# luofeisg/OpenKE-PuTransE

Hardware: AMD Instinct MI355X
Metric: training triples/sec (pos+neg) (higher is better)
Workload: dtype fp32; 1 GPU; C2 TransE fb15k237-shaped dim 200 p2 sgd lr 1 margin 5 batch 2000 neg 25 bern 1 filter 1 threads 8; global_batch=52000, parallelism=single

## Files before the change

include/putranse.h:

```cpp
#ifndef PUTRANSE_H
#define PUTRANSE_H
#include <stdint.h>

#ifdef __cplusplus
extern "C" {
#endif

enum {
    PT_OK = 0,
    PT_EINVAL = 1,
    PT_EIO = 2,
    PT_ENOMEM = 3,
    PT_EHIP = 4,
    PT_ESTATE = 5,
    PT_ENOTSUP = 6
};
const char *pt_last_error(void);
int pt_version(void);

typedef struct pt_graph pt_graph;
int pt_graph_load(const char *in_path, pt_graph **out);
int pt_set_count_header(int on);
int pt_get_count_header(void);
int pt_graph_free(pt_graph *g);
// ... 31 lines not shown

typedef struct pt_trainer pt_trainer;
int pt_trainer_create(const pt_model_desc *m, pt_trainer **out);
int pt_trainer_free(pt_trainer *t);
int pt_trainer_update_desc(pt_trainer *t, const pt_model_desc *m);
int pt_trainer_step(pt_trainer *t, pt_sampler *sampler, int64_t bs, int64_t neg, int64_t bern, int64_t filter,
                    const int64_t *d_batch_h, const int64_t *d_batch_t, const int64_t *d_batch_r, float *d_loss,
                    void *stream);
int pt_trainer_run(pt_trainer *t, pt_sampler *sampler, int64_t bs, int64_t neg, int64_t bern, int64_t filter,
                   int64_t steps, float *d_losses, void *stream);
int pt_trainer_fused_supported(const pt_trainer *t, int64_t bs, int64_t neg);

int pt_trainer_set_sampling(pt_trainer *t, int32_t path, int64_t parts);
int pt_trainer_set_positive_caps(pt_trainer *t, int32_t ent_cap, int32_t rel_cap);
int pt_trainer_positive_caps(const pt_trainer *t, int32_t *ent_cap, int32_t *rel_cap);
int pt_trainer_set_sample_split(pt_trainer *t, int64_t head);
int pt_trainer_set_deterministic(pt_trainer *t, int32_t on);
int pt_trainer_get_deterministic(const pt_trainer *t);

enum { PT_LOSS_MARGIN = 0, PT_LOSS_SIGMOID = 1 };
typedef struct {
    int32_t kind;
    int32_t adv;
    float temperature;
    int32_t score_margin_flag;
    float score_margin;
} pt_loss_desc;
int pt_trainer_set_loss(pt_trainer *t, const pt_loss_desc *loss);
typedef struct {
    float *ent_m, *rel_m, *norm_m;
// ... 13 lines not shown
                           const int64_t *d_batch_r, int64_t steps, float *d_loss, float *ms2, void *stream);

int pt_trainer_run_timed(pt_trainer *t, pt_sampler *sampler, int64_t bs, int64_t neg, int64_t bern, int64_t filter,
                         int64_t steps, float *d_losses, float *ms4, void *stream);
enum { PT_PATH_TWO_PASS = 0, PT_PATH_FUSED = 1, PT_PATH_PART = 2, PT_PATH_SAMPLED = 3 };
int pt_trainer_last_path(const pt_trainer *t);
int pt_trainer_set_step_apply(pt_trainer *t, int32_t on);
int pt_trainer_step_apply(const pt_trainer *t);
int pt_trainer_set_slot_scale(pt_trainer *t, int32_t on);
int pt_trainer_slot_scale(const pt_trainer *t);
int pt_trainer_sample_csr(pt_trainer *t, pt_sampler *sampler, int64_t bs, int64_t neg, int64_t bern, int64_t filter,
                          int64_t calls, int32_t path, int32_t *h_pos, int32_t *h_neg, int32_t *h_dst,
                          int32_t *h_start, void *stream);
int pt_trainer_positive_slots(pt_trainer *t, int64_t calls, int32_t *h_pdst, int32_t *h_pstart, int32_t *stored,
                              void *stream);

int pt_score(const pt_model_desc *m, int32_t mode, const int64_t *d_h, const int64_t *d_t, const int64_t *d_r,
             int64_t n, float *d_out, void *stream);

int pt_score_queries(const pt_model_desc *m, int32_t side, const int64_t *d_qh, const int64_t *d_qt,
                     const int64_t *d_qr, int64_t nq, float *d_out, void *stream);
int pt_score_rows(const pt_model_desc *m, int32_t side, const int64_t *d_qh, const int64_t *d_qt,
                  const int64_t *d_qr, int64_t nq, float *d_out, void *stream);
int pt_lp_metrics(const int64_t *rank_head, const int64_t *frank_head, const int64_t *rank_tail,
                  const int64_t *frank_tail, int64_t n, float *metrics);

typedef struct pt_universe pt_universe;
int pt_universe_build(const pt_graph *g, int64_t seed, int64_t threads, int64_t triple_constraint,
                      float balance, pt_universe **out);
int pt_universe_free(pt_universe *u);
// ... 163 lines not shown
```

openke-putranse_amd/csrc/apply.hip:

```cpp
#include <hip/hip_runtime.h>

#include <cstdint>

#include "device.h"
#include "graph.h"
#include "kernels.h"
#include "rng.h"

namespace pt {
namespace dev {
using pt::CsrWork;

struct ApplyTable {
    float *w, *acc, *grad;
    int *flag;
    int64_t rows;
    int jacobian;
    const int *start;
    const int *pstart;
};
struct ApplyParams {
    ApplyTable t[3];
    int ntab;
    int64_t dim;
    int opt;
    float lr;
    uint64_t *states;
    int64_t threads, bs, dpp;
    float *loss;
    const float *lpart;
    float margin, inv_count;
    int loss_assign;
    const float *contrib;
};

__device__ __forceinline__ void apply_block0(const ApplyParams &A) {
    const int lane = (int)threadIdx.x;
    if (A.states) advance_states(A.states, A.threads, A.bs, A.dpp, lane);
    if (A.loss && A.lpart) {
        float s = 0.f;
        for (int64_t i0 = lane; i0 < A.bs; i0 += 64 * 8) {
            float v[8];
#pragma unroll
            for (int u = 0; u < 8; ++u) v[u] = i0 + u * 64 < A.bs ? A.lpart[i0 + u * 64] : 0.f;
#pragma unroll
            for (int u = 0; u < 8; ++u) s += v[u];
        }
        s = gsum<64>(s);
// ... 61 lines not shown
        for (int i = 0; i < Vec::N; ++i) {
            a.x[i] = a.x[i] + g.x[i] * g.x[i];
            x.x[i] = x.x[i] + (-A.lr) * g.x[i] / (sqrtf(a.x[i]) + 1e-10f);
        }
        vstore(a, T.acc + row * D, D, lane);
    }
    vstore(x, T.w + row * D, D, lane);
    if (flagged) {
        Vec z;
        vzero(z);
        vstore(z, T.grad + row * D, D, lane);
        if (lane == 0) T.flag[row] = 0;
    }
}

template <int G, int VEC, int KCH, int NC>
__global__ __launch_bounds__(256) void k_apply_buf(ApplyParams A) {
    using Vec = V<G, VEC, KCH>;
    constexpr int GPB = 256 / G;
    const int lane = threadIdx.x % G;
    const int64_t gi = uni<G>((int32_t)(blockIdx.x * GPB + threadIdx.x / G));
    if (blockIdx.x == 0 && threadIdx.x < 64) apply_block0(A);
    const int D = (int)A.dim;
    const uint32_t rowb = (uint32_t)D * 4u;
    int64_t row = gi;
    int ti = 0;
    while (ti < A.ntab && row >= A.t[ti].rows) {
        row -= A.t[ti].rows;
        ++ti;
    }
    const bool live = ti < A.ntab;
    int flag = 0, c0 = 0, c1 = 0, p0 = 0, p1 = 0;
    Vec x, g, a;
#pragma unroll
    for (int once = 0; once < 1; ++once) {
        if (!live) continue;
        const ApplyTable &T = A.t[ti];
        const uint32_t tb = (uint32_t)T.rows * rowb;
        bload(x, make_rsrc(T.w, tb), (uint32_t)row * rowb, D, lane);
        if (A.opt != 0) bload(a, make_rsrc(T.acc, tb), (uint32_t)row * rowb, D, lane);
        flag = T.flag[row];
        if (T.start) {
            c0 = T.start[row];
            c1 = T.start[row + 1];
        }
        if (T.pstart) {
            p0 = T.pstart[row];
            p1 = T.pstart[row + 1];
        }
    }
    int len = 0, n0 = 0;
#pragma unroll
    for (int once = 0; once < 1; ++once) {
        if (!live) continue;
        const ApplyTable &T = A.t[ti];
        bload(g, make_rsrc(T.grad, (uint32_t)T.rows * rowb), flag ? (uint32_t)row * rowb : kOob, D, lane);
        n0 = c1 - c0;
        len = n0 + (p1 - p0);
    }
    const auto c_rs = make_rsrc(A.contrib, 0x7fffffffu);
    for (int j = 0; j < len; j += NC) {
        Vec c[NC];
#pragma unroll
        for (int q = 0; q < NC; ++q) {
            const int i = j + q;
            const int r = i < n0 ? c0 + i : p0 + (i - n0);
            bload(c[q], c_rs, i < len ? (uint32_t)r * rowb : kOob, D, lane);
        }
#pragma unroll
        for (int q = 0; q < NC; ++q)
#pragma unroll
            for (int i = 0; i < Vec::N; ++i) g.x[i] += c[q].x[i];
    }
#pragma unroll
    for (int once = 0; once < 1; ++once) {
        if (!live || (!flag && len == 0)) continue;
        const ApplyTable &T = A.t[ti];
        const uint32_t tb = (uint32_t)T.rows * rowb;
        Vec gg;
        if (T.jacobian) {
            const float n = sqrtf(vdot(x, x));
            vnormalize_bwd(x, n, g, gg);
        } else {
            gg = g;
        }
        if (A.opt == 0) {
#pragma unroll
// ... 21 lines not shown
hipError_t launch_apply(const StepParams &P, const StepWorkspace &W, uint64_t *states, int64_t threads, int64_t bs,
                        int64_t dpp, float *loss, hipStream_t st, const CsrWork *csr) {
    const Shape s = pick_shape(P.dim);
    dev::ApplyParams A{};
    A.ntab = 0;
    const int ent_j = P.model == 0 && P.norm_flag;
    const dev::ApplyTable ent{P.ent, P.ent_acc, W.gent, W.fent, P.ent_total, ent_j, csr ? csr->start : nullptr,
                              csr ? csr->pstart : nullptr};
    const dev::ApplyTable rel{P.rel, P.rel_acc, W.grel, W.frel, P.rel_total, P.norm_flag, nullptr,
                              csr && csr->pstart ? csr->pstart + P.ent_total : nullptr};
    A.t[A.ntab++] = csr ? rel : ent;
    A.t[A.ntab++] = csr ? ent : rel;
    if (P.model == 1)
        A.t[A.ntab++] = dev::ApplyTable{P.normv, P.norm_acc, W.gnorm, W.fnorm, P.rel_total, 1, nullptr, nullptr};
    A.contrib = csr ? csr->contrib : nullptr;
    A.dim = P.dim;
    A.opt = P.opt;
    A.lr = P.lr;
    A.states = states;
    A.threads = threads;
    A.bs = bs;
    A.dpp = dpp;
    A.loss = loss;
    A.lpart = W.lpart;
    A.margin = P.margin;
    A.inv_count = P.inv_count;
    A.loss_assign = P.loss_assign;
    int64_t rows = 0;
    for (int i = 0; i < A.ntab; ++i) rows += A.t[i].rows;
    const bool buf = P.dim % 4 == 0 && offsets_fit31(P, csr ? csr_con_rows(P.batch_size, P.neg) : 0);
    const int64_t gpb = 256 / s.G;
    const dim3 grid((unsigned)((rows + gpb - 1) / gpb)), block(256);
    hipError_t e = hipErrorInvalidValue;
    for_shape(s, [&](auto sh) {
        using T = decltype(sh);
        if constexpr (T::VEC == 4) {
            constexpr int NC = T::G == 64 && T::KCH == 1 ? 8 : 4;
            if (buf) {
                hipLaunchKernelGGL((dev::k_apply_buf<T::G, 4, T::KCH, NC>), grid, block, 0, st, A);
                e = hipGetLastError();
                return;
            }
        }
        hipLaunchKernelGGL((dev::k_apply<T::G, T::VEC, T::KCH>), grid, block, 0, st, A);
        e = hipGetLastError();
    });
    return e;
}

}
```

openke-putranse_amd/csrc/kernels.h:

```cpp
#pragma once
#include <hip/hip_runtime.h>

#include <cstdint>
#include <type_traits>

#include "graph.h"

namespace pt {

struct StepParams {
    int model, p_norm, norm_flag, opt;
    float lr, margin;
    int64_t ent_total, rel_total, dim;
    float *ent, *rel, *normv;
    float *ent_acc, *rel_acc, *norm_acc;
    int64_t batch_size, neg;
    float inv_count;
    int loss_assign = 0;
    float *ent_t = nullptr, *rel_t = nullptr;
    float *ent_t_acc = nullptr, *rel_t_acc = nullptr;
    float phase_div = 0.f;
};

struct StepWorkspace {
// ... 5 lines not shown
};

struct CsrWork {
    int4 *pos = nullptr;
    int32_t *neg = nullptr;
    int32_t *off = nullptr;
    int32_t *cnt = nullptr;
    int32_t *start = nullptr;
    float *contrib = nullptr;
    int32_t *tick = nullptr;
    int rank_only = 0;
    int64_t cnt_stride = 0, start_stride = 0;
    int4 *pdst = nullptr;
    int32_t *pstart = nullptr;
    int64_t pstart_stride = 0;
};

inline CsrWork csr_view(const CsrWork &w, int64_t call, int64_t bs, int64_t neg) {
    CsrWork v = w;
    v.pos = w.pos + call * bs;
    v.neg = w.neg + call * bs * neg;
    v.off = w.off + call * bs * neg;
    v.cnt = w.cnt + call * w.cnt_stride;
    v.start = w.start + call * w.start_stride;
    v.pdst = w.pdst + call * bs;
    v.pstart = w.pstart + call * w.pstart_stride;
    return v;
}

struct LpUniverseDev {
// ... 73 lines not shown
hipError_t launch_sample_part(const DeviceGraph &g, uint64_t *states, int64_t threads, int64_t bs, int64_t neg,
                              int bern, int filter, int64_t calls, int64_t parts, int64_t n, const CsrWork &w,
                              hipStream_t st);
bool sample_sort_prepare(int64_t bs, int64_t neg, int64_t n, int64_t start_stride);
bool sample_part_fits(int64_t bs, int64_t neg, int64_t n, int64_t parts);
bool sample_part_prepare(int64_t bs, int64_t neg, int64_t n, int64_t parts);
hipError_t launch_scan_counts(const CsrWork &w, int64_t n, int64_t calls, uint64_t *states, int64_t threads,
                              int64_t bs, int64_t dpp, hipStream_t st);
bool pos_slots_prepare(int64_t bs, int64_t neg, int64_t ent_total, int64_t rel_total);
hipError_t launch_pos_slots(const CsrWork &w, int64_t bs, int64_t neg, int64_t ent_total, int64_t rel_total,
                            int ent_cap, int rel_cap, int64_t calls, hipStream_t st);
inline bool offsets_fit31(const StepParams &P, int64_t con_rows) {
    return (P.ent_total + P.rel_total + con_rows) * P.dim * 4 < (int64_t(1) << 31);
}
inline int64_t csr_con_rows(int64_t bs, int64_t neg) { return bs * (neg + 3); }
bool csr_fast_path(const StepParams &P);
bool step_fits(const StepParams &P, int64_t neg, bool csr);
hipError_t launch_step(const StepParams &P, const DeviceGraph &g, const uint64_t *states, int64_t threads, int bern,
                       int filter, const int64_t *bh, const int64_t *bt, const int64_t *br, const StepWorkspace &W,
                       float *loss, hipStream_t st, const CsrWork *csr = nullptr);
hipError_t launch_apply(const StepParams &P, const StepWorkspace &W, uint64_t *states, int64_t threads, int64_t bs,
                        int64_t dpp, float *loss, hipStream_t st, const CsrWork *csr = nullptr);
struct LossParams {
    int kind = 0, adv = 0;
    float temp = 0.f;
    int mflag = 0;
    float gamma = 0.f;
    bool plain() const { return kind == 0 && !adv && !mflag; }
};
inline void loss_affine(const LossParams &L, const StepParams &P, float *scale, float *cst) {
// ... 83 lines not shown
```

openke-putranse_amd/csrc/step.hip:

```cpp
#include <hip/hip_runtime.h>

#include <cstdint>

#include "device.h"
#include "graph.h"
#include "kernels.h"
#include "rng.h"

namespace pt {
namespace dev {
using pt::CsrWork;

struct GlobalSink {
    float *gent, *grel, *gnorm;
    int *fent, *frel, *fnorm;
    float *lpart;
    template <int G, int VEC, int KCH>
    __device__ __forceinline__ void ent(int64_t row, const V<G, VEC, KCH> &g, int D, int lane) const {
        vatomic(g, gent + row * D, D, lane);
        if (lane == 0) fent[row] = 1;
    }
    template <int G, int VEC, int KCH>
    __device__ __forceinline__ void rel(int64_t row, const V<G, VEC, KCH> &g, int D, int lane) const {
        vatomic(g, grel + row * D, D, lane);
// ... 264 lines not shown
    constexpr int PPB = GPB / S;
    constexpr int RW = KCH * G * VEC;
    __shared__ float red[S > 1 ? GPB * 2 * RW + 2 * GPB : 1];
    __shared__ float trb[PPB * 3 * RW];
    const int lane = threadIdx.x % G;
    const int grp = threadIdx.x / G;
    const int sub = grp % S;
    const int64_t b = (int64_t)blockIdx.x * PPB + grp / S;
    const bool active = b < P.batch_size;
    const int D = (int)P.dim;
    const uint32_t rowb = (uint32_t)D * 4u;
    const int neg = (int)P.neg;
    constexpr int p = PN;
    const bool nf = P.norm_flag != 0;
    const float m = P.margin, inv = P.inv_count;
    const int nper = (neg + S - 1) / S;
    const int k_lo = sub * nper < neg ? sub * nper : neg;
    const int k_hi = k_lo + nper < neg ? k_lo + nper : neg;
    Vec At, Ah, rh, th, bt;
    vzero(At); vzero(Ah); vzero(rh); vzero(th); vzero(bt);
    float csum = 0.f, lsum = 0.f, ps = 0.f;
    int32_t hp = 0, rp = 0, tp = 0;
    int32_t dh = -1, dr = -1, dt = -1;
    const uint32_t conb = (uint32_t)(P.batch_size * (neg + 3)) * rowb;
    if (active) {
        const auto ent_rs = make_rsrc(P.ent, (uint32_t)P.ent_total * rowb);
        const auto rel_rs = make_rsrc(P.rel, (uint32_t)P.rel_total * rowb);
        const auto con_rs = make_rsrc(cw.contrib, conb);
        const int4 q = cw.pos[b];
        const int4 qd = cw.pdst[b];
        hp = uni<G>(q.x); rp = uni<G>(q.y); tp = uni<G>(q.z);
        dh = uni<G>(qd.x); dr = uni<G>(qd.y); dt = uni<G>(qd.z);
        const int32_t *nrec = cw.neg + b * neg;
        const int32_t *ndst = cw.off + b * neg;
        int w0 = k_lo, wend = k_hi - k_lo < G ? k_hi : k_lo + G;
        int32_t rec = 0, dst = 0;
        if (w0 + lane < wend) {
            rec = nrec[w0 + lane];
            dst = ndst[w0 + lane];
            if (cw.rank_only) dst += cw.start[rec >> 1];
        }
        Vec H, T, Rr;
        bload(H, ent_rs, (uint32_t)hp * rowb, D, lane);
        bload(T, ent_rs, (uint32_t)tp * rowb, D, lane);
        bload(Rr, rel_rs, (uint32_t)rp * rowb, D, lane);
        Vec EA[NCH], EB[NCH];
        auto load_chunk = [&](Vec(&E)[NCH], int k0) {
#pragma unroll
            for (int u = 0; u < NCH; ++u) {
                const int kk = k0 + u < wend ? k0 + u : wend - 1;
                const uint32_t e = (uint32_t)(gbcast<G>(rec, kk - w0) >> 1);
                bload(E[u], ent_rs, e * rowb, D, lane);
            }
        };
        if (w0 < wend) load_chunk(EA, w0);
        Vec hh, vpos;
        if (nf) {
            vnormalize<true>(H, hh);
            vnormalize<true>(Rr, rh);
            vnormalize<true>(T, th);
        } else {
            hh = H; rh = Rr; th = T;
        }
#pragma unroll
        for (int i = 0; i < Vec::N; ++i) {
            bt.x[i] = hh.x[i] + rh.x[i];
            vpos.x[i] = bt.x[i] - th.x[i];
        }
        ps = vpnorm<true>(vpos, p);
        auto process = [&](Vec(&E)[NCH], int k0) {
#pragma unroll
            for (int u = 0; u < NCH; ++u) {
                if (k0 + u < wend) {
                const int32_t r = gbcast<G>(rec, k0 + u - w0);
                const int32_t di = gbcast<G>(dst, k0 + u - w0);
                const uint32_t slot = (uint32_t)di * rowb;
                const bool tail_side = r & 1;
                Vec eh, vk, gs;
                if (nf) vnormalize<true>(E[u], eh); else eh = E[u];
                if (tail_side) {
#pragma unroll
                    for (int i = 0; i < Vec::N; ++i) vk.x[i] = bt.x[i] - eh.x[i];
                } else {
#pragma unroll
                    for (int i = 0; i < Vec::N; ++i) vk.x[i] = (eh.x[i] + rh.x[i]) - th.x[i];
                }
                const float ns = vpnorm<true>(vk, p);
                const float a = uni<G>(ps - ns);
                lsum += a > -m ? a : -m;
                const float c = a > -m ? inv : (a == -m ? inv * 0.5f : 0.f);
                csum += c;
                vpnorm_bwd<true>(vk, ns, p, tail_side ? c : -c, gs);
                bstore(gs, con_rs, slot, D, lane);
                if (tail_side) {
#pragma unroll
                    for (int i = 0; i < Vec::N; ++i) At.x[i] -= gs.x[i];
                } else {
#pragma unroll
                    for (int i = 0; i < Vec::N; ++i) Ah.x[i] += gs.x[i];
                }
                }
            }
        };
        while (w0 < wend) {
            for (int c0 = w0; c0 < wend;) {
                if (c0 + NCH < wend) load_chunk(EB, c0 + NCH);
                process(EA, c0);
                c0 += NCH;
                if (c0 >= wend) break;
                if (c0 + NCH < wend) load_chunk(EA, c0 + NCH);
                process(EB, c0);
                c0 += NCH;
            }
            w0 = wend;
            if (w0 >= k_hi) break;
            wend = k_hi - w0 < G ? k_hi : w0 + G;
            rec = dst = 0;
            if (w0 + lane < wend) {
                rec = nrec[w0 + lane];
                dst = ndst[w0 + lane];
                if (cw.rank_only) dst += cw.start[rec >> 1];
            }
            load_chunk(EA, w0);
        }
    }
    if constexpr (S > 1) {
        float *mr = red + grp * 2 * RW;
#pragma unroll
        for (int k = 0; k < Vec::N; ++k) {
            const int c = ((k / VEC) * G + lane) * VEC + k % VEC;
            mr[c] = At.x[k];
            mr[RW + c] = Ah.x[k];
        }
        float *cs = red + GPB * 2 * RW;
        if (lane == 0) {
            cs[grp * 2 + 0] = csum;
// ... 86 lines not shown
    X(4, 1, 1, 1, 1) X(4, 1, 1, 4, 1) X(4, 1, 1, 8, 1) X(4, 1, 1, 8, 4) X(4, 1, 1, 32, 4)             \
    X(8, 1, 1, 1, 1) X(8, 1, 1, 4, 1) X(8, 1, 1, 8, 1) X(8, 1, 1, 8, 4) X(8, 1, 1, 32, 4)             \
    X(16, 1, 1, 1, 1) X(16, 1, 1, 4, 1) X(16, 1, 1, 8, 1) X(16, 1, 1, 8, 4) X(16, 1, 1, 32, 4)        \
    X(32, 1, 1, 1, 1) X(32, 1, 1, 4, 1) X(32, 1, 1, 8, 1) X(32, 1, 1, 8, 4) X(32, 1, 1, 32, 4)        \
    X(64, 1, 1, 1, 1) X(64, 1, 1, 4, 1) X(64, 1, 1, 8, 1) X(64, 1, 1, 8, 4) X(64, 1, 1, 32, 4)        \
    X(64, 1, 2, 1, 1) X(64, 1, 2, 4, 1) X(64, 1, 2, 8, 1) X(64, 1, 2, 8, 4) X(64, 1, 2, 32, 4)        \
    X(64, 1, 4, 1, 1) X(64, 1, 4, 4, 1) X(64, 1, 4, 8, 1) X(64, 1, 4, 8, 4) X(64, 1, 4, 32, 4)        \
    X(64, 1, 4, 4, 4)                                                                                 \
    X(64, 1, 8, 1, 1) X(64, 1, 8, 4, 1) X(64, 1, 8, 8, 1) X(64, 1, 8, 8, 4)

}
static constexpr int kCsrNch = 2;
constexpr int csr_nch(int kch, int s) { return kch >= 4 && s == 1 ? 1 : kCsrNch; }

bool csr_fast_path(const StepParams &P) {
    return P.model == 0 && P.dim % 4 == 0 && offsets_fit31(P, csr_con_rows(P.batch_size, P.neg));
}

bool step_fits(const StepParams &P0, int64_t neg, bool csr) {
    StepParams P = P0;
    P.neg = neg;
    if (csr && csr_fast_path(P)) return true;
    if (!narrow_dim_supported(P.dim)) return false;
    const Shape s = pick_shape(P.dim, false);
    const int S = (neg >= 8 && 256 / s.G >= 4) ? 4 : 1;
    const int64_t gpb = 256 / s.G, ppb = gpb / S;
    size_t lds = (size_t)ppb * (size_t)neg * sizeof(int64_t) * (csr ? 2 : 1);
    if (S > 1) lds += sizeof(float) * ((size_t)gpb * 4 * s.KCH * s.G * s.VEC + (size_t)gpb * 2);
    return lds <= 64 * 1024;
}

hipError_t launch_step(const StepParams &P, const DeviceGraph &g, const uint64_t *states, int64_t threads, int bern,
                       int filter, const int64_t *bh, const int64_t *bt, const int64_t *br, const StepWorkspace &W,
                       float *loss, hipStream_t st, const CsrWork *csr) {
    if (P.batch_size <= 0) return hipSuccess;
    dev::GlobalSink sink{W.gent, W.grel, W.gnorm, W.fent, W.frel, W.fnorm, W.lpart};
    hipError_t e = hipErrorInvalidValue;
    if (bh) {
        const Shape s = pick_shape(P.dim);
        const int64_t gpb = 256 / s.G;
        const dim3 grid((unsigned)((P.batch_size + gpb - 1) / gpb)), block(256);
        for_shape(s, [&](auto sh) {
            for_value<0, 1>(P.model != 0, [&](auto m) {
                using T = decltype(sh);
                hipLaunchKernelGGL((dev::k_step<m.value, T::G, T::VEC, T::KCH>), grid, block, 0, st, P, bh, bt, br, sink,
                                   loss);
                e = hipGetLastError();
            });
        });
        return e;
    }
    if (csr && csr_fast_path(P)) {
        const Shape s = pick_shape(P.dim);
        int S = 1;
        while (S < 4 && S * 2 <= 256 / s.G && P.neg >= 6 * S * 2) S *= 2;
        const bool matched = for_shape(s, [&](auto sh) {
            using T = decltype(sh);
            if constexpr (T::VEC == 4)
                for_value<1, 2, 4>(S, [&](auto sv) {
                    for_value<1, 2>(P.p_norm == 1 ? 1 : 2, [&](auto pn) {
                        constexpr int SG = sv.value * T::G, NT = SG >= 256 || 256 % SG != 0 ? SG : 256;
                        const dim3 grid((unsigned)((P.batch_size * SG + NT - 1) / NT)), block(NT);
                        constexpr int NCH = csr_nch(T::KCH, sv.value);
                        hipLaunchKernelGGL((dev::k_step_csr<T::G, 4, T::KCH, NCH, sv.value, pn.value, NT>), grid, block,
                                           0, st, P, sink, *csr);
                        e = hipGetLastError();
                    });
// ... 37 lines not shown
```

openke-putranse_amd/csrc/trainer.cpp:

```cpp
#include <algorithm>
#include <cmath>
#include <map>
#include <memory>
#include <string>
#include <tuple>
#include <vector>

#include "common.h"
#include "graph.h"
#include "kernels.h"
#include "ordered.h"
#include "trainer.h"

struct GraphKey {
    const void *sampler, *graph, *losses, *states;
    int64_t bs, neg, bern, filter, steps;
    bool operator<(const GraphKey &o) const {
        return std::tie(sampler, graph, losses, states, bs, neg, bern, filter, steps) <
               std::tie(o.sampler, o.graph, o.losses, o.states, o.bs, o.neg, o.bern, o.filter, o.steps);
    }
};

static const int32_t kDefaultEntCap = 8, kDefaultRelCap = 32;

// ... 5 lines not shown
    void *csr_block = nullptr;
    size_t csr_cap = 0;
    pt::CsrWork csr{};
    int64_t csr_bs = 0, csr_neg = 0, csr_chunk = 0;
    bool csr_fused = false;
    bool csr_part = false;
    int last_path = -1;
    int64_t lpart_cap = 0;
    int device = -1;
    hipStream_t cap = nullptr;
    std::map<GraphKey, hipGraphExec_t> graphs;
    int path_override = -1;
    int64_t parts_override = 0;
    int32_t ent_cap_set = -1, rel_cap_set = -1;
    bool pos_stored = false;
    int32_t ent_cap() const { return !pos_stored ? 0 : ent_cap_set < 0 ? kDefaultEntCap : ent_cap_set; }
    int32_t rel_cap() const { return !pos_stored ? 0 : rel_cap_set < 0 ? kDefaultRelCap : rel_cap_set; }
    bool ordered = false;
    void *ord_block = nullptr;
    size_t ord_cap = 0;
    int64_t *ord_h = nullptr, *ord_t = nullptr, *ord_r = nullptr;
    float *ord_y = nullptr, *ord_score = nullptr, *ord_ds = nullptr;
    float *ord_g = nullptr;
    pt::LossParams loss{};
    pt::AdamParams adam{};
    bool adam_set = false;
    int64_t adam_step = 0;
    pt::RegulParams regul{};
    float *l3part = nullptr;
    bool extended() const {
// ... 105 lines not shown
static int choose_path(const pt_trainer *t, int64_t calls, int64_t bs, int64_t neg, int forced) {
    const bool part_ok = t->csr_part && pt::sample_part_fits(bs, neg, t->P.ent_total, part_count(t, calls, bs));
    if (forced == PT_PATH_FUSED && t->csr_fused) return PT_PATH_FUSED;
    if (forced == PT_PATH_PART && part_ok) return PT_PATH_PART;
    if (forced == PT_PATH_TWO_PASS) return PT_PATH_TWO_PASS;
    if (t->csr_fused && calls >= kSampleSortMinCalls) return PT_PATH_FUSED;
    if (part_ok) return PT_PATH_PART;
    return PT_PATH_TWO_PASS;
}

static int ensure_csr(pt_trainer *t, int64_t bs, int64_t neg) {
    if (t->csr_block && t->csr_bs == bs && t->csr_neg == neg) return PT_OK;
    const int64_t E = t->P.ent_total, R = t->P.rel_total, D = t->P.dim;
    const int64_t cs = (E + 3) & ~int64_t(3), ss = (E + 4) & ~int64_t(3), ps = (E + R + 4) & ~int64_t(3);
    auto al = [](size_t b) { return (b + 255) & ~size_t(255); };
    const size_t per_call = 32 * bs + 8 * bs * neg + 4 * cs + 4 * ss + 4 * ps + 4 + 1024;
    const int64_t chunk = std::min<int64_t>(kCsrChunk, (int64_t)std::max<size_t>(1, ((size_t)512 << 20) / per_call));
    const size_t a_pos = al(16 * bs * chunk), a_neg = al(4 * bs * neg * chunk), a_off = a_neg,
                 a_cnt = al(4 * cs * chunk), a_start = al(4 * ss * chunk), a_tick = al(4 * chunk + 4),
                 a_con = al(4 * pt::csr_con_rows(bs, neg) * D), a_pdst = a_pos, a_pstart = al(4 * ps * chunk);
    const size_t need = a_pos + a_neg + a_off + a_cnt + a_start + a_tick + a_con + a_pdst + a_pstart;
    PT_HIP(hipDeviceSynchronize());
    t->drop_graphs();
    if (need > t->csr_cap) {
        if (t->csr_block) (void)hipFree(t->csr_block);
        t->csr_block = nullptr;
        t->csr_cap = 0;
        PT_HIP(hipMalloc(&t->csr_block, need));
        t->csr_cap = need;
    }
    PT_HIP(hipMemset(t->csr_block, 0, need));
    char *b = (char *)t->csr_block;
    t->csr.pos = (int4 *)b; b += a_pos;
    t->csr.neg = (int32_t *)b; b += a_neg;
    t->csr.off = (int32_t *)b; b += a_off;
    t->csr.cnt = (int32_t *)b; b += a_cnt;
    t->csr.start = (int32_t *)b; b += a_start;
    t->csr.tick = (int32_t *)b; b += a_tick;
    t->csr.contrib = (float *)b; b += a_con;
    t->csr.pdst = (int4 *)b; b += a_pdst;
    t->csr.pstart = (int32_t *)b;
    t->csr.cnt_stride = cs;
    t->csr.start_stride = ss;
    t->csr.pstart_stride = ps;
    PT_HIP(hipMemset(t->csr.pdst, 0xff, a_pdst));
    PT_HIP(hipMemsetD32((hipDeviceptr_t)t->csr.pstart, (int)(bs * neg), (size_t)(ps * chunk)));
    t->csr_bs = bs;
    t->csr_neg = neg;
    t->csr_chunk = chunk;
    t->csr_fused = pt::sample_sort_prepare(bs, neg, E, ss);
    t->csr_part = pt::sample_part_prepare(bs, neg, E, std::min<int64_t>(bs, kPartTarget));
    pt::StepParams Q = t->P;
    Q.batch_size = bs;
    Q.neg = neg;
    t->pos_stored = pt::csr_fast_path(Q) && pt::pos_slots_prepare(bs, neg, E, R);
    return PT_OK;
}

struct Timing {
    std::vector<hipEvent_t> pool;
    size_t used = 0;
    std::vector<std::tuple<int, hipEvent_t, hipEvent_t>> ev;
    int reserve(size_t n) {
        pool.resize(n);
        for (auto &e : pool) PT_HIP(hipEventCreate(&e));
        return PT_OK;
    }
    int begin(int kind, hipStream_t st, hipEvent_t *a) {
        if (used >= pool.size()) return pt::fail(PT_EHIP, "timing event pool exhausted");
        *a = pool[used++];
// ... 278 lines not shown
    PT_CHECK(ent_cap >= -1 && rel_cap >= -1, PT_EINVAL, "positive caps must be >= 0, or -1 for the library's choice");
    PT_HIP(hipDeviceSynchronize());
    t->ent_cap_set = ent_cap;
    t->rel_cap_set = rel_cap;
    t->drop_graphs();
    t->csr_bs = 0;
    return PT_OK;
}
extern "C" int pt_trainer_positive_caps(const pt_trainer *t, int32_t *ent_cap, int32_t *rel_cap) {
    PT_CHECK(t && ent_cap && rel_cap, PT_EINVAL, "pt_trainer_positive_caps: null argument");
    *ent_cap = t->ent_cap_set < 0 ? kDefaultEntCap : t->ent_cap_set;
    *rel_cap = t->rel_cap_set < 0 ? kDefaultRelCap : t->rel_cap_set;
    return PT_OK;
}

extern "C" int pt_trainer_set_deterministic(pt_trainer *t, int32_t on) {
    PT_CHECK(t, PT_EINVAL, "null trainer");
    PT_CHECK(!on || pt::ordered_dim_supported(t->P.dim), PT_ENOTSUP, "reference-order mode: dim too large");
    PT_CHECK(!on || t->P.model != PT_TRANSD, PT_ENOTSUP, "reference-order mode is not implemented for TransD");
    PT_CHECK(!on || t->P.model != PT_ROTATE, PT_ENOTSUP, "reference-order mode is not implemented for PT_ROTATE");
    PT_CHECK(!on || t->P.model != PT_DISTMULT, PT_ENOTSUP, "reference-order mode is not implemented for PT_DISTMULT");
    PT_CHECK(!on || t->P.model != PT_COMPLEX, PT_ENOTSUP, "reference-order mode is not implemented for PT_COMPLEX");
    t->ordered = on != 0;
    return PT_OK;
}
extern "C" int pt_trainer_get_deterministic(const pt_trainer *t) { return t && t->ordered ? 1 : 0; }

extern "C" int pt_trainer_set_loss(pt_trainer *t, const pt_loss_desc *l) {
    PT_CHECK(t && l, PT_EINVAL, "pt_trainer_set_loss: null argument");
    PT_CHECK(l->kind == PT_LOSS_MARGIN || l->kind == PT_LOSS_SIGMOID, PT_EINVAL,
// ... 272 lines not shown
    const int64_t bs = t->csr_bs, n = t->P.ent_total + t->P.rel_total + 1;
    std::vector<int4> d((size_t)(calls * bs));
    PT_HIP(hipMemcpyAsync(d.data(), w.pdst, sizeof(int4) * d.size(), hipMemcpyDeviceToHost, st));
    PT_HIP(hipMemcpy2DAsync(h_pstart, 4 * (size_t)n, w.pstart, 4 * (size_t)w.pstart_stride, 4 * (size_t)n, (size_t)calls,
                            hipMemcpyDeviceToHost, st));
    PT_HIP(hipStreamSynchronize(st));
    for (size_t i = 0; i < d.size(); ++i) {
        h_pdst[3 * i] = d[i].x;
        h_pdst[3 * i + 1] = d[i].y;
        h_pdst[3 * i + 2] = d[i].z;
    }
    *stored = t->pos_stored ? 1 : 0;
    return PT_OK;
}

extern "C" int pt_trainer_fused_supported(const pt_trainer *t, int64_t bs, int64_t neg) {
    return t && fused_supported(t, bs, neg) ? 1 : 0;
}

extern "C" int pt_trainer_run(pt_trainer *t, pt_sampler *s, int64_t bs, int64_t neg, int64_t bern, int64_t filter,
                              int64_t steps, float *d_losses, void *stream) {
    PT_CHECK(t && d_losses, PT_EINVAL, "pt_trainer_run: null argument");
    PT_CHECK(steps > 0, PT_EINVAL, "steps must be positive");
    PT_CHECK(!t->extended(), PT_ENOTSUP, kExtendedMsg);
    if (t->ordered) {
        PT_CHECK(bs > 0 && neg > 0, PT_EINVAL, "batch_size and neg_ent must be positive");
        return enqueue_ordered_run(t, s, bs, neg, bern, filter, steps, d_losses, 1, (hipStream_t)stream);
    }
    int rc = prepare_sampled(t, s, bs, neg);
    if (rc) return rc;
// ... 20 lines not shown
```

openke-putranse_amd/openke/_native.py:

```python
import ctypes
import os

_HERE = os.path.dirname(os.path.abspath(__file__))
LIB_PATH = os.path.join(_HERE, "release", "libputranse_hip.so")
_LIB = None
_ALTERNATIVE = False

c_i64 = ctypes.c_int64
c_i32 = ctypes.c_int32
c_f32 = ctypes.c_float
c_vp = ctypes.c_void_p
c_u64p = ctypes.POINTER(ctypes.c_uint64)
c_i64p = ctypes.POINTER(ctypes.c_int64)
c_f32p = ctypes.POINTER(ctypes.c_float)

PT_TRANSE, PT_TRANSH, PT_TRANSD, PT_ROTATE, PT_DISTMULT, PT_COMPLEX = 0, 1, 2, 3, 4, 5
PT_SGD, PT_ADAGRAD, PT_ADAM = 0, 1, 2
PT_LOSS_MARGIN, PT_LOSS_SIGMOID = 0, 1
PT_DETERMINISTIC = 1
PT_PATH_TWO_PASS, PT_PATH_FUSED, PT_PATH_PART, PT_PATH_SAMPLED = 0, 1, 2, 3
PATH_KERNELS = {PT_PATH_TWO_PASS: ("k_sample_csr", "k_scan_counts"), PT_PATH_FUSED: ("k_sample_sort", "k_advance"),
                PT_PATH_PART: ("k_sample_part", None), PT_PATH_SAMPLED: (None, None)}


# ... 68 lines not shown
    "pt_sampler_sample": (ctypes.c_int, [c_vp, c_i64, c_i64, c_i64, c_i64, c_vp, c_vp, c_vp, c_vp, c_vp]),
    "pt_sampler_sample_ex": (ctypes.c_int, [c_vp, c_i64, c_i64, c_i64, c_i64, c_i64, c_i64, c_vp, c_vp, c_vp, c_vp,
                                            c_vp]),
    "pt_trainer_create": (ctypes.c_int, [ctypes.POINTER(ModelDesc), ctypes.POINTER(c_vp)]),
    "pt_trainer_free": (ctypes.c_int, [c_vp]),
    "pt_trainer_update_desc": (ctypes.c_int, [c_vp, ctypes.POINTER(ModelDesc)]),
    "pt_trainer_step": (ctypes.c_int, [c_vp, c_vp, c_i64, c_i64, c_i64, c_i64, c_vp, c_vp, c_vp, c_vp, c_vp]),
    "pt_trainer_run": (ctypes.c_int, [c_vp, c_vp, c_i64, c_i64, c_i64, c_i64, c_i64, c_vp, c_vp]),
    "pt_trainer_run_timed": (ctypes.c_int, [c_vp, c_vp, c_i64, c_i64, c_i64, c_i64, c_i64, c_vp, c_vp, c_vp]),
    "pt_trainer_last_path": (ctypes.c_int, [c_vp]),
    "pt_trainer_set_deterministic": (ctypes.c_int, [c_vp, c_i32]),
    "pt_trainer_set_sampling": (ctypes.c_int, [c_vp, c_i32, c_i64]),
    "pt_trainer_set_positive_caps": (ctypes.c_int, [c_vp, c_i32, c_i32]),
    "pt_trainer_positive_caps": (ctypes.c_int, [c_vp, ctypes.POINTER(c_i32), ctypes.POINTER(c_i32)]),
    "pt_trainer_positive_slots": (ctypes.c_int, [c_vp, c_i64, c_vp, c_vp, ctypes.POINTER(c_i32), c_vp]),
    "pt_trainer_set_sample_split": (ctypes.c_int, [c_vp, c_i64]),
    "pt_trainer_set_step_apply": (ctypes.c_int, [c_vp, c_i32]),
    "pt_universe_dim_supported": (ctypes.c_int, [c_i64, c_i32]),
    "pt_model_dim_supported": (ctypes.c_int, [c_i64, c_i32]),
    "pt_trainer_fused_supported": (ctypes.c_int, [c_vp, c_i64, c_i64]),
    "pt_trainer_step_apply": (ctypes.c_int, [c_vp]),
    "pt_trainer_get_deterministic": (ctypes.c_int, [c_vp]),
    "pt_trainer_set_loss": (ctypes.c_int, [c_vp, ctypes.POINTER(LossDesc)]),
    "pt_trainer_set_adam": (ctypes.c_int, [c_vp, ctypes.POINTER(AdamState)]),
    "pt_trainer_set_regul": (ctypes.c_int, [c_vp, ctypes.POINTER(RegulDesc)]),
    "pt_trainer_adam_step": (c_i64, [c_vp]),
    "pt_trainer_steps_timed": (ctypes.c_int, [c_vp, c_i64, c_i64, c_vp, c_vp, c_vp, c_i64, c_vp, c_vp, c_vp]),
    "pt_trainer_sample_csr": (ctypes.c_int, [c_vp, c_vp, c_i64, c_i64, c_i64, c_i64, c_i64, ctypes.c_int32, c_vp,
                                             c_vp, c_vp, c_vp, c_vp]),
    "pt_score": (ctypes.c_int, [ctypes.POINTER(ModelDesc), c_i32, c_vp, c_vp, c_vp, c_i64, c_vp, c_vp]),
# ... 151 lines not shown
```

Measured before the change: 1.682 billion triples/s.

## Replace per-negative gradient rows with compact records rebuilt in apply kernel

The step kernel no longer writes a full dim-wide gradient row per negative sample into the contrib buffer. Each negative now stores an 8-byte record (batch index, side bit, scalar coefficient) into a per-entity slot table, plus two per-triple base vectors (h+r and r-t). The apply kernel reconstructs each negative gradient from the base vector and the entity's normalized embedding, cutting write and read traffic on the contrib buffer. Negatives beyond a per-entity cap, chosen from the mean plus 4 sigma of the sampling count, fall back to atomic adds into the entity gradient. This adds register pressure, extra normalization work in apply, and an atomic path whose cost depends on overflow frequency.

```diff
diff --git a/include/putranse.h b/include/putranse.h
--- a/include/putranse.h
+++ b/include/putranse.h
@@ -69,6 +69,8 @@
 int pt_trainer_set_sampling(pt_trainer *t, int32_t path, int64_t parts);
 int pt_trainer_set_positive_caps(pt_trainer *t, int32_t ent_cap, int32_t rel_cap);
 int pt_trainer_positive_caps(const pt_trainer *t, int32_t *ent_cap, int32_t *rel_cap);
+int pt_trainer_set_negative_cap(pt_trainer *t, int32_t cap);
+int pt_trainer_negative_cap(const pt_trainer *t, int32_t *cap);
 int pt_trainer_set_sample_split(pt_trainer *t, int64_t head);
 int pt_trainer_set_deterministic(pt_trainer *t, int32_t on);
 int pt_trainer_get_deterministic(const pt_trainer *t);
@@ -112,6 +114,7 @@
                           int32_t *h_start, void *stream);
 int pt_trainer_positive_slots(pt_trainer *t, int64_t calls, int32_t *h_pdst, int32_t *h_pstart, int32_t *stored,
                               void *stream);
+int pt_trainer_negative_records(pt_trainer *t, int32_t *h_rec, int64_t capacity, int32_t *cap, void *stream);
 
 int pt_score(const pt_model_desc *m, int32_t mode, const int64_t *d_h, const int64_t *d_t, const int64_t *d_r,
              int64_t n, float *d_out, void *stream);
diff --git a/openke-putranse_amd/csrc/apply.hip b/openke-putranse_amd/csrc/apply.hip
--- a/openke-putranse_amd/csrc/apply.hip
+++ b/openke-putranse_amd/csrc/apply.hip
@@ -32,6 +32,11 @@
     float margin, inv_count;
     int loss_assign;
     const float *contrib;
+    const int2 *nrec;
+    int32_t ncap;
+    uint32_t base_off;
+    uint32_t base_rowb;
+    int p_norm;
 };
 
 __device__ __forceinline__ void apply_block0(const ApplyParams &A) {
@@ -123,7 +128,8 @@
     }
 }
 
-template <int G, int VEC, int KCH, int NC>
+typedef __attribute__((address_space(4))) i32x4 crec4;
+template <int G, int VEC, int KCH, int NC, bool REC = false>
 __global__ __launch_bounds__(256) void k_apply_buf(ApplyParams A) {
     using Vec = V<G, VEC, KCH>;
     constexpr int GPB = 256 / G;
@@ -141,6 +147,7 @@
     const bool live = ti < A.ntab;
     int flag = 0, c0 = 0, c1 = 0, p0 = 0, p1 = 0;
     Vec x, g, a;
+    i32x4 R[REC ? NC / 2 : 1] = {};
 #pragma unroll
     for (int once = 0; once < 1; ++once) {
         if (!live) continue;
@@ -157,6 +164,13 @@
             p0 = T.pstart[row];
             p1 = T.pstart[row + 1];
         }
+        if constexpr (REC) {
+            if (T.start && A.ncap > 0) {
+                const crec4 *rp = (const crec4 *)(uintptr_t)(A.nrec + row * A.ncap);
+#pragma unroll
+                for (int q = 0; q < NC / 2; ++q) R[q] = rp[q];
+            }
+        }
     }
     int len = 0, n0 = 0;
 #pragma unroll
@@ -165,21 +179,66 @@
         const ApplyTable &T = A.t[ti];
         bload(g, make_rsrc(T.grad, (uint32_t)T.rows * rowb), flag ? (uint32_t)row * rowb : kOob, D, lane);
         n0 = c1 - c0;
+        if constexpr (REC) n0 = n0 < A.ncap ? n0 : A.ncap;
         len = n0 + (p1 - p0);
     }
     const auto c_rs = make_rsrc(A.contrib, 0x7fffffffu);
-    for (int j = 0; j < len; j += NC) {
-        Vec c[NC];
-#pragma unroll
-        for (int q = 0; q < NC; ++q) {
-            const int i = j + q;
-            const int r = i < n0 ? c0 + i : p0 + (i - n0);
-            bload(c[q], c_rs, i < len ? (uint32_t)r * rowb : kOob, D, lane);
-        }
-#pragma unroll
-        for (int q = 0; q < NC; ++q)
-#pragma unroll
-            for (int i = 0; i < Vec::N; ++i) g.x[i] += c[q].x[i];
+    if constexpr (!REC) {
+        for (int j = 0; j < len; j += NC) {
+            Vec c[NC];
+#pragma unroll
+            for (int q = 0; q < NC; ++q) {
+                const int i = j + q;
+                const int r = i < n0 ? c0 + i : p0 + (i - n0);
+                bload(c[q], c_rs, i < len ? (uint32_t)r * rowb : kOob, D, lane);
+            }
+#pragma unroll
+            for (int q = 0; q < NC; ++q)
+#pragma unroll
+                for (int i = 0; i < Vec::N; ++i) g.x[i] += c[q].x[i];
+        }
+    } else {
+        Vec eh;
+        vzero(eh);
+        for (int j = 0; j < len; j += NC) {
+            if (j > 0 && j < n0) {
+                const crec4 *rp = (const crec4 *)(uintptr_t)(A.nrec + row * A.ncap + j);
+#pragma unroll
+                for (int q = 0; q < NC / 2; ++q) R[q] = rp[q];
+            }
+            Vec c[NC];
+#pragma unroll
+            for (int q = 0; q < NC; ++q) {
+                const int i = j + q;
+                const int32_t slot = q % 2 ? R[q / 2].z : R[q / 2].x;
+                const uint32_t off = i < n0 ? A.base_off + (uint32_t)(slot ^ 1) * A.base_rowb
+                                            : (uint32_t)(p0 + (i - n0)) * rowb;
+                bload(c[q], c_rs, i < len ? off : kOob, D, lane);
+            }
+            if (j == 0 && n0 > 0) {
+                if (A.t[ti].jacobian) vnormalize<true>(x, eh); else eh = x;
+            }
+#pragma unroll
+            for (int q = 0; q < NC; ++q) {
+#pragma clang fp contract(off)
+                const int i = j + q;
+                const int32_t slot = q % 2 ? R[q / 2].z : R[q / 2].x;
+                const float k = __int_as_float(q % 2 ? R[q / 2].w : R[q / 2].y);
+                if (i < n0) {
+                    const float s = slot & 1 ? -1.f : 1.f;
+#pragma unroll
+                    for (int e = 0; e < Vec::N; ++e) {
+                        const float v = __builtin_fmaf(s, eh.x[e], c[q].x[e]);
+                        float kv;
+                        if (A.p_norm == 1) kv = v > 0.f ? k : (v < 0.f ? -k : 0.f); else kv = k * v;
+                        g.x[e] = g.x[e] + kv;
+                    }
+                } else {
+#pragma unroll
+                    for (int e = 0; e < Vec::N; ++e) g.x[e] += c[q].x[e];
+                }
+            }
+        }
     }
 #pragma unroll
     for (int once = 0; once < 1; ++once) {
@@ -231,6 +290,14 @@
     if (P.model == 1)
         A.t[A.ntab++] = dev::ApplyTable{P.normv, P.norm_acc, W.gnorm, W.fnorm, P.rel_total, 1, nullptr, nullptr};
     A.contrib = csr ? csr->contrib : nullptr;
+    const bool rec = csr && csr->ncap >= 0 && csr_fast_path(P);
+    if (rec) {
+        A.nrec = csr->nrec;
+        A.ncap = csr->ncap;
+        A.base_off = (uint32_t)((const char *)csr->bases - (const char *)csr->contrib);
+        A.base_rowb = (uint32_t)csr->bstride * 4u;
+        A.p_norm = P.p_norm;
+    }
     A.dim = P.dim;
     A.opt = P.opt;
     A.lr = P.lr;
@@ -254,7 +321,10 @@
         if constexpr (T::VEC == 4) {
             constexpr int NC = T::G == 64 && T::KCH == 1 ? 8 : 4;
             if (buf) {
-                hipLaunchKernelGGL((dev::k_apply_buf<T::G, 4, T::KCH, NC>), grid, block, 0, st, A);
+                if (rec)
+                    hipLaunchKernelGGL((dev::k_apply_buf<T::G, 4, T::KCH, NC, true>), grid, block, 0, st, A);
+                else
+                    hipLaunchKernelGGL((dev::k_apply_buf<T::G, 4, T::KCH, NC>), grid, block, 0, st, A);
                 e = hipGetLastError();
                 return;
             }
diff --git a/openke-putranse_amd/csrc/kernels.h b/openke-putranse_amd/csrc/kernels.h
--- a/openke-putranse_amd/csrc/kernels.h
+++ b/openke-putranse_amd/csrc/kernels.h
@@ -43,6 +43,10 @@
     int4 *pdst = nullptr;
     int32_t *pstart = nullptr;
     int64_t pstart_stride = 0;
+    float *bases = nullptr;
+    int2 *nrec = nullptr;
+    int32_t ncap = -1;
+    int32_t bstride = 0;
 };
 
 inline CsrWork csr_view(const CsrWork &w, int64_t call, int64_t bs, int64_t neg) {
@@ -146,6 +150,14 @@
     return (P.ent_total + P.rel_total + con_rows) * P.dim * 4 < (int64_t(1) << 31);
 }
 inline int64_t csr_con_rows(int64_t bs, int64_t neg) { return bs * (neg + 3); }
+constexpr int32_t kMaxNegCap = 64;
+inline int64_t base_row_stride(int64_t dim) { return dim; }
+inline bool records_fit31(const StepParams &P) {
+    const int64_t con = 4 * csr_con_rows(P.batch_size, P.neg) * P.dim + 256;
+    return con + 8 * P.batch_size * base_row_stride(P.dim) < (int64_t(1) << 31) &&
+           P.ent_total * kMaxNegCap * 8 < (int64_t(1) << 31);
+}
+int32_t default_negative_cap(const StepParams &P);
 bool csr_fast_path(const StepParams &P);
 bool step_fits(const StepParams &P, int64_t neg, bool csr);
 hipError_t launch_step(const StepParams &P, const DeviceGraph &g, const uint64_t *states, int64_t threads, int bern,
diff --git a/openke-putranse_amd/csrc/step.hip b/openke-putranse_amd/csrc/step.hip
--- a/openke-putranse_amd/csrc/step.hip
+++ b/openke-putranse_amd/csrc/step.hip
@@ -1,5 +1,6 @@
 #include <hip/hip_runtime.h>
 
+#include <cmath>
 #include <cstdint>
 
 #include "device.h"
@@ -302,19 +303,21 @@
     constexpr int p = PN;
     const bool nf = P.norm_flag != 0;
     const float m = P.margin, inv = P.inv_count;
+    const int32_t cap = cw.ncap;
     const int nper = (neg + S - 1) / S;
     const int k_lo = sub * nper < neg ? sub * nper : neg;
     const int k_hi = k_lo + nper < neg ? k_lo + nper : neg;
-    Vec At, Ah, rh, th, bt;
-    vzero(At); vzero(Ah); vzero(rh); vzero(th); vzero(bt);
+    Vec At, Ah, bh, th, bt;
+    vzero(At); vzero(Ah); vzero(bh); vzero(th); vzero(bt);
     float csum = 0.f, lsum = 0.f, ps = 0.f;
     int32_t hp = 0, rp = 0, tp = 0;
     int32_t dh = -1, dr = -1, dt = -1;
     const uint32_t conb = (uint32_t)(P.batch_size * (neg + 3)) * rowb;
+    float *ob = S > 1 ? red + grp * 2 * RW : trb + grp * 3 * RW;
     if (active) {
         const auto ent_rs = make_rsrc(P.ent, (uint32_t)P.ent_total * rowb);
         const auto rel_rs = make_rsrc(P.rel, (uint32_t)P.rel_total * rowb);
-        const auto con_rs = make_rsrc(cw.contrib, conb);
+        const auto rec_rs = make_rsrc(cw.nrec, (uint32_t)P.ent_total * (uint32_t)cap * 8u);
         const int4 q = cw.pos[b];
         const int4 qd = cw.pdst[b];
         hp = uni<G>(q.x); rp = uni<G>(q.y); tp = uni<G>(q.z);
@@ -322,11 +325,11 @@
         const int32_t *nrec = cw.neg + b * neg;
         const int32_t *ndst = cw.off + b * neg;
         int w0 = k_lo, wend = k_hi - k_lo < G ? k_hi : k_lo + G;
-        int32_t rec = 0, dst = 0;
+        int32_t rec = 0, rank = 0;
         if (w0 + lane < wend) {
             rec = nrec[w0 + lane];
-            dst = ndst[w0 + lane];
-            if (cw.rank_only) dst += cw.start[rec >> 1];
+            rank = ndst[w0 + lane];
+            if (!cw.rank_only) rank -= cw.start[rec >> 1];
         }
         Vec H, T, Rr;
         bload(H, ent_rs, (uint32_t)hp * rowb, D, lane);
@@ -342,53 +345,103 @@
             }
         };
         if (w0 < wend) load_chunk(EA, w0);
-        Vec hh, vpos;
-        if (nf) {
-            vnormalize<true>(H, hh);
-            vnormalize<true>(Rr, rh);
-            vnormalize<true>(T, th);
-        } else {
-            hh = H; rh = Rr; th = T;
-        }
-#pragma unroll
-        for (int i = 0; i < Vec::N; ++i) {
-            bt.x[i] = hh.x[i] + rh.x[i];
-            vpos.x[i] = bt.x[i] - th.x[i];
-        }
-        ps = vpnorm<true>(vpos, p);
+        {
+            Vec hh, rh, vpos;
+            if (nf) {
+                vnormalize<true>(H, hh);
+                vnormalize<true>(Rr, rh);
+                vnormalize<true>(T, th);
+            } else {
+                hh = H; rh = Rr; th = T;
+            }
+#pragma unroll
+            for (int i = 0; i < Vec::N; ++i) {
+                bt.x[i] = hh.x[i] + rh.x[i];
+                bh.x[i] = rh.x[i] - th.x[i];
+                vpos.x[i] = bt.x[i] - th.x[i];
+            }
+            ps = vpnorm<true>(vpos, p);
+        }
+        if (sub == 0) {
+            const uint32_t bsb = (uint32_t)cw.bstride * 4u;
+            const auto bas_rs = make_rsrc(cw.bases, (uint32_t)P.batch_size * 2u * bsb);
+            bstore(bt, bas_rs, (uint32_t)b * 2u * bsb, D, lane);
+            bstore(bh, bas_rs, ((uint32_t)b * 2u + 1u) * bsb, D, lane);
+        }
+        float kmine = 0.f;
         auto process = [&](Vec(&E)[NCH], int k0) {
 #pragma unroll
             for (int u = 0; u < NCH; ++u) {
                 if (k0 + u < wend) {
+#pragma clang fp contract(off)
                 const int32_t r = gbcast<G>(rec, k0 + u - w0);
-                const int32_t di = gbcast<G>(dst, k0 + u - w0);
-                const uint32_t slot = (uint32_t)di * rowb;
                 const bool tail_side = r & 1;
-                Vec eh, vk, gs;
+                Vec eh, vk;
                 if (nf) vnormalize<true>(E[u], eh); else eh = E[u];
                 if (tail_side) {
 #pragma unroll
                     for (int i = 0; i < Vec::N; ++i) vk.x[i] = bt.x[i] - eh.x[i];
                 } else {
 #pragma unroll
-                    for (int i = 0; i < Vec::N; ++i) vk.x[i] = (eh.x[i] + rh.x[i]) - th.x[i];
+                    for (int i = 0; i < Vec::N; ++i) vk.x[i] = eh.x[i] + bh.x[i];
                 }
                 const float ns = vpnorm<true>(vk, p);
                 const float a = uni<G>(ps - ns);
                 lsum += a > -m ? a : -m;
                 const float c = a > -m ? inv : (a == -m ? inv * 0.5f : 0.f);
                 csum += c;
-                vpnorm_bwd<true>(vk, ns, p, tail_side ? c : -c, gs);
-                bstore(gs, con_rs, slot, D, lane);
+                const float ds = tail_side ? c : -c;
+                float kk;
+                if constexpr (p == 1) kk = ds; else kk = ns == 0.f ? 0.f : ds * frcp<true>(ns);
+                kk = uni<G>(kk);
+                if (lane == k0 + u - w0) kmine = kk;
+                auto gsi = [&](int i) {
+                    if constexpr (p == 1) return vk.x[i] > 0.f ? kk : (vk.x[i] < 0.f ? -kk : 0.f); else return kk * vk.x[i];
+                };
                 if (tail_side) {
 #pragma unroll
-                    for (int i = 0; i < Vec::N; ++i) At.x[i] -= gs.x[i];
+                    for (int i = 0; i < Vec::N; ++i) At.x[i] -= gsi(i);
                 } else {
 #pragma unroll
-                    for (int i = 0; i < Vec::N; ++i) Ah.x[i] += gs.x[i];
-                }
-                }
-            }
+                    for (int i = 0; i < Vec::N; ++i) Ah.x[i] += gsi(i);
+                }
+                }
+            }
+        };
+        auto overflow_slots = [&]() {
+            const int32_t over = w0 + lane < wend && rank >= cap && kmine != 0.f ? 1 : 0;
+            if (gsum<G>((float)over) == 0.f) return;
+            for (int j = 0; j < wend - w0; ++j) {
+#pragma clang fp contract(off)
+                if (!gbcast<G>(over, j)) continue;
+                const int32_t r = gbcast<G>(rec, j);
+                const float kk = __int_as_float(gbcast<G>(__float_as_int(kmine), j));
+                const int64_t e = r >> 1;
+                Vec Ev, eh;
+                bload(Ev, ent_rs, (uint32_t)e * rowb, D, lane);
+                if (nf) vnormalize<true>(Ev, eh); else eh = Ev;
+                __builtin_amdgcn_wave_barrier();
+#pragma unroll
+                for (int k = 0; k < Vec::N; ++k) {
+                    const float v = r & 1 ? bt.x[k] - eh.x[k] : eh.x[k] + bh.x[k];
+                    float gk;
+                    if constexpr (p == 1) gk = v > 0.f ? kk : (v < 0.f ? -kk : 0.f); else gk = kk * v;
+                    ob[((k / VEC) * G + lane) * VEC + k % VEC] = gk;
+                }
+                __builtin_amdgcn_wave_barrier();
+                float *ge = sink.gent + e * D;
+#pragma unroll 1
+                for (int c2 = lane; c2 < D; c2 += G) atomicAdd(ge + c2, ob[c2]);
+                if (lane == 0) sink.fent[e] = 1;
+                __builtin_amdgcn_wave_barrier();
+            }
+        };
+        auto store_records = [&]() {
+            const bool mine = w0 + lane < wend && rank < cap;
+            const uint32_t off = mine ? ((uint32_t)(rec >> 1) * (uint32_t)cap + (uint32_t)rank) * 8u : kOob;
+            typedef unsigned int u32x2 __attribute__((ext_vector_type(2)));
+            const u32x2 v = {((uint32_t)b << 1) | (uint32_t)(rec & 1), __float_as_uint(kmine)};
+            __builtin_amdgcn_raw_buffer_store_b64(v, rec_rs, off, 0, 0);
         };
         while (w0 < wend) {
             for (int c0 = w0; c0 < wend;) {
@@ -400,14 +453,16 @@
                 process(EB, c0);
                 c0 += NCH;
             }
+            store_records();
+            overflow_slots();
             w0 = wend;
             if (w0 >= k_hi) break;
             wend = k_hi - w0 < G ? k_hi : w0 + G;
-            rec = dst = 0;
+            rec = rank = 0;
             if (w0 + lane < wend) {
                 rec = nrec[w0 + lane];
-                dst = ndst[w0 + lane];
-                if (cw.rank_only) dst += cw.start[rec >> 1];
+                rank = ndst[w0 + lane];
+                if (!cw.rank_only) rank -= cw.start[rec >> 1];
             }
             load_chunk(EA, w0);
         }
@@ -524,13 +579,10 @@
 constexpr int csr_nch(int kch, int s) { return kch >= 4 && s == 1 ? 1 : kCsrNch; }
 
 bool csr_fast_path(const StepParams &P) {
-    return P.model == 0 && P.dim % 4 == 0 && offsets_fit31(P, csr_con_rows(P.batch_size, P.neg));
-}
-
-bool step_fits(const StepParams &P0, int64_t neg, bool csr) {
-    StepParams P = P0;
-    P.neg = neg;
-    if (csr && csr_fast_path(P)) return true;
+    return P.model == 0 && P.dim % 4 == 0 && offsets_fit31(P, csr_con_rows(P.batch_size, P.neg)) && records_fit31(P);
+}
+
+static bool sampled_fits(const StepParams &P, int64_t neg, bool csr) {
     if (!narrow_dim_supported(P.dim)) return false;
     const Shape s = pick_shape(P.dim, false);
     const int S = (neg >= 8 && 256 / s.G >= 4) ? 4 : 1;
@@ -538,6 +590,22 @@
     size_t lds = (size_t)ppb * (size_t)neg * sizeof(int64_t) * (csr ? 2 : 1);
     if (S > 1) lds += sizeof(float) * ((size_t)gpb * 4 * s.KCH * s.G * s.VEC + (size_t)gpb * 2);
     return lds <= 64 * 1024;
+}
+
+int32_t default_negative_cap(const StepParams &P) {
+    const double mean = (double)P.batch_size * (double)P.neg / (double)(P.ent_total > 0 ? P.ent_total : 1);
+    const double bound = mean + 4.0 * std::sqrt(mean);
+    int32_t cap = 8;
+    while (cap < kMaxNegCap && cap < bound) cap += 8;
+    if (cap < bound && sampled_fits(P, P.neg, true)) return -1;
+    return cap;
+}
+
+bool step_fits(const StepParams &P0, int64_t neg, bool csr) {
+    StepParams P = P0;
+    P.neg = neg;
+    if (csr && csr_fast_path(P)) return true;
+    return sampled_fits(P, neg, csr);
 }
 
 hipError_t launch_step(const StepParams &P, const DeviceGraph &g, const uint64_t *states, int64_t threads, int bern,
@@ -560,7 +628,7 @@
         });
         return e;
     }
-    if (csr && csr_fast_path(P)) {
+    if (csr && csr->ncap >= 0 && csr_fast_path(P)) {
         const Shape s = pick_shape(P.dim);
         int S = 1;
         while (S < 4 && S * 2 <= 256 / s.G && P.neg >= 6 * S * 2) S *= 2;
diff --git a/openke-putranse_amd/csrc/trainer.cpp b/openke-putranse_amd/csrc/trainer.cpp
--- a/openke-putranse_amd/csrc/trainer.cpp
+++ b/openke-putranse_amd/csrc/trainer.cpp
@@ -43,6 +43,7 @@
     int64_t parts_override = 0;
     int32_t ent_cap_set = -1, rel_cap_set = -1;
     bool pos_stored = false;
+    int32_t neg_cap_set = -1;
     int32_t ent_cap() const { return !pos_stored ? 0 : ent_cap_set < 0 ? kDefaultEntCap : ent_cap_set; }
     int32_t rel_cap() const { return !pos_stored ? 0 : rel_cap_set < 0 ? kDefaultRelCap : rel_cap_set; }
     bool ordered = false;
@@ -178,12 +179,19 @@
     const int64_t E = t->P.ent_total, R = t->P.rel_total, D = t->P.dim;
     const int64_t cs = (E + 3) & ~int64_t(3), ss = (E + 4) & ~int64_t(3), ps = (E + R + 4) & ~int64_t(3);
     auto al = [](size_t b) { return (b + 255) & ~size_t(255); };
+    pt::StepParams Q = t->P;
+    Q.batch_size = bs;
+    Q.neg = neg;
+    const bool fast = pt::csr_fast_path(Q);
+    const int32_t ncap = !fast ? -1 : t->neg_cap_set >= 0 ? t->neg_cap_set : pt::default_negative_cap(Q);
+    const int64_t bstride = pt::base_row_stride(D);
     const size_t per_call = 32 * bs + 8 * bs * neg + 4 * cs + 4 * ss + 4 * ps + 4 + 1024;
     const int64_t chunk = std::min<int64_t>(kCsrChunk, (int64_t)std::max<size_t>(1, ((size_t)512 << 20) / per_call));
     const size_t a_pos = al(16 * bs * chunk), a_neg = al(4 * bs * neg * chunk), a_off = a_neg,
                  a_cnt = al(4 * cs * chunk), a_start = al(4 * ss * chunk), a_tick = al(4 * chunk + 4),
-                 a_con = al(4 * pt::csr_con_rows(bs, neg) * D), a_pdst = a_pos, a_pstart = al(4 * ps * chunk);
-    const size_t need = a_pos + a_neg + a_off + a_cnt + a_start + a_tick + a_con + a_pdst + a_pstart;
+                 a_con = al(4 * pt::csr_con_rows(bs, neg) * D), a_pdst = a_pos, a_pstart = al(4 * ps * chunk),
+                 a_bas = ncap >= 0 ? al(8 * bs * bstride) : 0, a_rec = ncap > 0 ? al(8 * E * ncap) : 0;
+    const size_t need = a_pos + a_neg + a_off + a_cnt + a_start + a_tick + a_con + a_bas + a_rec + a_pdst + a_pstart;
     PT_HIP(hipDeviceSynchronize());
     t->drop_graphs();
     if (need > t->csr_cap) {
@@ -202,6 +210,10 @@
     t->csr.start = (int32_t *)b; b += a_start;
     t->csr.tick = (int32_t *)b; b += a_tick;
     t->csr.contrib = (float *)b; b += a_con;
+    t->csr.bases = (float *)b; b += a_bas;
+    t->csr.nrec = (int2 *)b; b += a_rec;
+    t->csr.ncap = ncap;
+    t->csr.bstride = (int32_t)bstride;
     t->csr.pdst = (int4 *)b; b += a_pdst;
     t->csr.pstart = (int32_t *)b;
     t->csr.cnt_stride = cs;
@@ -214,10 +226,7 @@
     t->csr_chunk = chunk;
     t->csr_fused = pt::sample_sort_prepare(bs, neg, E, ss);
     t->csr_part = pt::sample_part_prepare(bs, neg, E, std::min<int64_t>(bs, kPartTarget));
-    pt::StepParams Q = t->P;
-    Q.batch_size = bs;
-    Q.neg = neg;
-    t->pos_stored = pt::csr_fast_path(Q) && pt::pos_slots_prepare(bs, neg, E, R);
+    t->pos_stored = fast && ncap >= 0 && pt::pos_slots_prepare(bs, neg, E, R);
     return PT_OK;
 }
 
@@ -526,6 +535,22 @@
     return PT_OK;
 }
 
+extern "C" int pt_trainer_set_negative_cap(pt_trainer *t, int32_t cap) {
+    PT_CHECK(t, PT_EINVAL, "null trainer");
+    PT_CHECK(cap == -1 || (cap >= 0 && cap <= pt::kMaxNegCap && cap % 8 == 0), PT_EINVAL,
+             "negative cap must be 0, a multiple of 8 up to 64, or -1 for the library's choice");
+    PT_HIP(hipDeviceSynchronize());
+    t->neg_cap_set = cap;
+    t->drop_graphs();
+    t->csr_bs = 0;
+    return PT_OK;
+}
+extern "C" int pt_trainer_negative_cap(const pt_trainer *t, int32_t *cap) {
+    PT_CHECK(t && cap, PT_EINVAL, "pt_trainer_negative_cap: null argument");
+    *cap = t->neg_cap_set;
+    return PT_OK;
+}
+
 extern "C" int pt_trainer_set_deterministic(pt_trainer *t, int32_t on) {
     PT_CHECK(t, PT_EINVAL, "null trainer");
     PT_CHECK(!on || pt::ordered_dim_supported(t->P.dim), PT_ENOTSUP, "reference-order mode: dim too large");
@@ -828,6 +853,20 @@
     return PT_OK;
 }
 
+extern "C" int pt_trainer_negative_records(pt_trainer *t, int32_t *h_rec, int64_t capacity, int32_t *cap,
+                                           void *stream) {
+    PT_CHECK(t && cap, PT_EINVAL, "pt_trainer_negative_records: null argument");
+    PT_CHECK(t->csr_block, PT_ESTATE, "pt_trainer_negative_records: no counting-sort step was run");
+    *cap = t->csr.ncap;
+    if (t->csr.ncap <= 0) return PT_OK;
+    const int64_t n = 2 * t->P.ent_total * t->csr.ncap;
+    PT_CHECK(h_rec && capacity >= n, PT_EINVAL, "pt_trainer_negative_records: buffer too small");
+    hipStream_t st = (hipStream_t)stream;
+    PT_HIP(hipMemcpyAsync(h_rec, t->csr.nrec, 4 * (size_t)n, hipMemcpyDeviceToHost, st));
+    PT_HIP(hipStreamSynchronize(st));
+    return PT_OK;
+}
+
 extern "C" int pt_trainer_fused_supported(const pt_trainer *t, int64_t bs, int64_t neg) {
     return t && fused_supported(t, bs, neg) ? 1 : 0;
 }
diff --git a/openke-putranse_amd/openke/_native.py b/openke-putranse_amd/openke/_native.py
--- a/openke-putranse_amd/openke/_native.py
+++ b/openke-putranse_amd/openke/_native.py
@@ -106,6 +106,9 @@
     "pt_trainer_set_positive_caps": (ctypes.c_int, [c_vp, c_i32, c_i32]),
     "pt_trainer_positive_caps": (ctypes.c_int, [c_vp, ctypes.POINTER(c_i32), ctypes.POINTER(c_i32)]),
     "pt_trainer_positive_slots": (ctypes.c_int, [c_vp, c_i64, c_vp, c_vp, ctypes.POINTER(c_i32), c_vp]),
+    "pt_trainer_set_negative_cap": (ctypes.c_int, [c_vp, c_i32]),
+    "pt_trainer_negative_cap": (ctypes.c_int, [c_vp, ctypes.POINTER(c_i32)]),
+    "pt_trainer_negative_records": (ctypes.c_int, [c_vp, c_vp, c_i64, ctypes.POINTER(c_i32), c_vp]),
     "pt_trainer_set_sample_split": (ctypes.c_int, [c_vp, c_i64]),
     "pt_trainer_set_step_apply": (ctypes.c_int, [c_vp, c_i32]),
     "pt_universe_dim_supported": (ctypes.c_int, [c_i64, c_i32]),
```

Result: faster. 1.715 billion triples/s (median of 6 runs) (+1.9%).
